# nathanaelbosch/ODEFilters.jl

Hardware: AMD Instinct MI355X
Metric: ensemble ODE-filter steps/sec (whole node) (higher is better)
Workload: dtype f64

## Files before the change

### odefilters.jl_amd/csrc/smooth_lane.h

```cpp
#pragma once
#include "ek_lane.h"

namespace odef {

struct LaneMem {
  double* base;
  int stride;
  __device__ inline double get(int k) const { return base[k * stride]; }
  __device__ inline void set(int k, double v) const { base[k * stride] = v; }
};

template <int D>
__device__ inline void two_sided_inverse(double (&S)[D * (D + 1) / 2], const double (&L)[D * (D + 1) / 2], const double (&dinv)[D]) {
  static_for<0, D>([&](auto kc) {
    constexpr int k = decltype(kc)::value;
    const double inv = dinv[k];
    const double tkk = S[tri(k, k)] * inv * inv;
    S[tri(k, k)] = tkk;
    const double htkk = -0.5 * tkk;
#pragma unroll
    for (int j = 0; j < k; ++j) S[tri(k, j)] *= inv;
    double b[D];
#pragma unroll
    for (int i = k + 1; i < D; ++i) {
      const double lik = L[tri(i, k)];
      b[i] = __builtin_fma(lik, htkk, S[tri(i, k)] * inv);
#pragma unroll
      for (int j = 0; j < k; ++j) S[tri(i, j)] = __builtin_fma(-lik, S[tri(k, j)], S[tri(i, j)]);
    }
#pragma unroll
    for (int i = k + 1; i < D; ++i) {
      const double lik = L[tri(i, k)];
#pragma unroll
      for (int j = k + 1; j <= i; ++j)
        S[tri(i, j)] = __builtin_fma(-L[tri(j, k)], b[i], __builtin_fma(-lik, b[j], S[tri(i, j)]));
      S[tri(i, k)] = __builtin_fma(lik, htkk, b[i]);
    }
    ODEF_SCHED_FENCE();
  });
  static_for<0, D>([&](auto kc) {
    constexpr int k = D - 1 - decltype(kc)::value;
    const double inv = dinv[k];
    double t[D];
#pragma unroll
    for (int j = 0; j < D; ++j) {
      double s = S[symidx(k, j)];
#pragma unroll
      for (int i = k + 1; i < D; ++i) s -= L[tri(i, k)] * S[symidx(i, j)];
      t[j] = s;
    }
    double tk = t[k];
#pragma unroll
    for (int i = k + 1; i < D; ++i) tk -= L[tri(i, k)] * t[i];
#pragma unroll
    for (int j = 0; j < D; ++j)
      if (j != k) S[symidx(k, j)] = t[j] * inv;
    S[tri(k, k)] = tk * inv * inv;
    ODEF_SCHED_FENCE();
  });
}

template <int d, int NB>
__device__ inline void congruence_At_inplace(const PriorConsts& pc, double (&X)[d * NB * (d * NB + 1) / 2]) {
  constexpr int D = d * NB;
#pragma unroll
  for (int J = NB - 1; J >= 1; --J) {
    double Wd[d][d];
#pragma unroll
    for (int a = 0; a < d; ++a)
#pragma unroll
      for (int b = 0; b < d; ++b) {
        double t = X[symidx(J * d + a, J * d + b)];
#pragma unroll
        for (int j = 0; j < J; ++j) t += pc.At[j][J] * X[symidx(j * d + a, J * d + b)];
        Wd[a][b] = t;
      }
#pragma unroll
    for (int a = 0; a < d; ++a)
#pragma unroll
      for (int c = 0; c < D; ++c) {
        if (c / d == J) continue;
        double t = X[symidx(J * d + a, c)];
#pragma unroll
        for (int j = 0; j < J; ++j) t += pc.At[j][J] * X[symidx(j * d + a, c)];
        X[symidx(J * d + a, c)] = t;
      }
#pragma unroll
    for (int a = 0; a < d; ++a)
#pragma unroll
      for (int b = 0; b <= a; ++b) {
        double t = Wd[a][b];
#pragma unroll
        for (int j = 0; j < J; ++j) t += pc.At[j][J] * X[symidx(J * d + a, j * d + b)];
        X[tri(J * d + a, J * d + b)] = t;
      }
  }
}

template <int d, int NB, class CovSink, class Sig = double>
__device__ inline void rts_step_core(const PriorConsts& pc, const double (&pij)[NB], const double (&mt)[d * NB],
                                     double (&B)[d * NB * (d * NB + 1) / 2], double (&Cs)[d * NB * (d * NB + 1) / 2],
                                     const double (&msn)[d * NB], Sig sigma2, const LaneMem& xl,
                                     double (&ms_out)[d * NB], CovSink& sink) {
  constexpr int D = d * NB, TRI = D * (D + 1) / 2;
  double dl[D];
#pragma unroll
  for (int J = 0; J < NB; ++J)
#pragma unroll
    for (int a = 0; a < d; ++a) {
      double t = mt[J * d + a];
#pragma unroll
      for (int j = J + 1; j < NB; ++j) t += pc.At[J][j] * mt[j * d + a];
      dl[J * d + a] = msn[J * d + a] - t;
    }
  ODEF_SCHED_FENCE();
  predict_cov_inplace<d, NB>(pc, B, sigma2);
  ODEF_SCHED_FENCE();
#pragma unroll
  for (int k = 0; k < TRI; ++k) Cs[k] -= B[k];
  int fixes = 0;
  double dinv[D];
  chol_packed<D>(B, fixes, dinv);
  ODEF_SCHED_FENCE();
#pragma unroll
  for (int k = 0; k < D; ++k) {
    double t = dl[k];
#pragma unroll
    for (int c = 0; c < k; ++c) t -= B[tri(k, c)] * dl[c];
    dl[k] = t * dinv[k];
  }
#pragma unroll
  for (int k = D - 1; k >= 0; --k) {
    double t = dl[k];
#pragma unroll
    for (int c = k + 1; c < D; ++c) t -= B[tri(c, k)] * dl[c];
    dl[k] = t * dinv[k];
  }
  double wv[D];
#pragma unroll
  for (int K = 0; K < NB; ++K)
#pragma unroll
    for (int b = 0; b < d; ++b) {
      double t = dl[K * d + b];
#pragma unroll
      for (int j = 0; j < K; ++j) t += pc.At[j][K] * dl[j * d + b];
      wv[K * d + b] = t;
    }
  ODEF_SCHED_FENCE();
  two_sided_inverse<D>(Cs, B, dinv);
  ODEF_SCHED_FENCE();
  congruence_At_inplace<d, NB>(pc, Cs);
  ODEF_SCHED_FENCE();
  static_for<0, D>([&](auto ac) {
    constexpr int a = decltype(ac)::value;
    double xa[D], u[D];
#pragma unroll
    for (int c = 0; c < D; ++c) xa[c] = xl.get(symidx(a, c));
    double mnew = mt[a];
#pragma unroll
    for (int c = 0; c < D; ++c) mnew += xa[c] * wv[c];
    ms_out[a] = mnew * pij[a / d];
#pragma unroll
    for (int c = 0; c < D; ++c) {
      double t = 0.0;
#pragma unroll
      for (int k = 0; k < D; ++k) t += xa[k] * Cs[symidx(k, c)];
      u[c] = t;
    }
#pragma unroll
    for (int b = 0; b <= a; ++b) {
      double t = xa[b];
#pragma unroll
      for (int k = 0; k < D; ++k) t += u[k] * xl.get(symidx(k, b));
      sink(tri(a, b), t * (pij[a / d] * pij[b / d]));
    }
    ODEF_SCHED_FENCE();
  });
}

__device__ inline long wave_uniform_max(long v, bool valid) {
#ifdef ODEF_HOST_EMUL
  (void)valid;
  return v;
#else
  int x = valid ? (int)v : 0;
  for (int m = 32; m >= 1; m >>= 1) {
    const int y = __shfl_xor(x, m, 64);
    x = x > y ? x : y;
  }
  return (long)__builtin_amdgcn_readfirstlane(x);
#endif
}

#ifdef ODEF_HOST_EMUL
inline double* agpr_file() {
  static thread_local double f[256];
  return f;
}
template <int R>
inline void aput(double v) { agpr_file()[R] = v; }
template <int R>
inline double aget() { return agpr_file()[R]; }
inline void agpr_file_claim() {}
#else
template <int R>
__device__ __attribute__((always_inline)) inline void aput(double v) {
  static_assert(R >= 0 && R < 128, "a lane has 256 AGPRs = 128 doubles");
  asm volatile("v_accvgpr_write_b32 a[%1], %0" ::"v"(__double2loint(v)), "n"(2 * R));
  asm volatile("v_accvgpr_write_b32 a[%1], %0" ::"v"(__double2hiint(v)), "n"(2 * R + 1));
}
template <int R>
__device__ __attribute__((always_inline)) inline double aget() {
  static_assert(R >= 0 && R < 128, "a lane has 256 AGPRs = 128 doubles");
  int lo, hi;
  asm volatile("v_accvgpr_read_b32 %0, a[%1]" : "=v"(lo) : "n"(2 * R));
  asm volatile("v_accvgpr_read_b32 %0, a[%1]" : "=v"(hi) : "n"(2 * R + 1));
  return __hiloint2double(hi, lo);
}
__device__ __attribute__((always_inline)) inline void agpr_file_claim() { asm volatile("" ::: "a255"); }
#endif

template <int n>
__device__ __attribute__((always_inline)) inline void pin(double (&a)[n]) {
#ifndef ODEF_HOST_EMUL
#pragma unroll
  for (int k = 0; k < n; ++k) asm volatile("" : "+v"(a[k]));
#else
  (void)a;
#endif
}

template <int D>
__device__ inline void ldl_packed_lane(double (&B)[D * (D + 1) / 2], double (&dinv)[D]) {
  static_for<0, D>([&](auto kc) {
    constexpr int k = decltype(kc)::value;
    const double piv = B[tri(k, k)];
    const bool ok = piv > 0.0;
    const double inv = ok ? rcp_pos(ok ? piv : 1.0) : 0.0;
    dinv[k] = inv;
    double v[D];
#pragma unroll
    for (int i = k + 1; i < D; ++i) {
      v[i] = B[tri(i, k)];
      B[tri(i, k)] = v[i] * inv;
    }
#pragma unroll
    for (int j = k + 1; j < D; ++j)
#pragma unroll
      for (int i = j; i < D; ++i) B[tri(i, j)] = __builtin_fma(-B[tri(i, k)], v[j], B[tri(i, j)]);
  });
}

template <int D, int LS>
__device__ inline void two_sided_inverse_parked(double (&S)[D * (D + 1) / 2]) {
  static_for<0, D>([&](auto kc) {
    constexpr int k = decltype(kc)::value;
    double lc[D];
    static_for<k + 1, D>([&](auto ic) { lc[decltype(ic)::value] = aget<LS + tri(decltype(ic)::value, k)>(); });
    const double htkk = -0.5 * S[tri(k, k)];
    double b[D];
#pragma unroll
    for (int i = k + 1; i < D; ++i) {
      b[i] = __builtin_fma(lc[i], htkk, S[tri(i, k)]);
#pragma unroll
      for (int j = 0; j < k; ++j) S[tri(i, j)] = __builtin_fma(-lc[i], S[tri(k, j)], S[tri(i, j)]);
    }
#pragma unroll
    for (int i = k + 1; i < D; ++i) {
#pragma unroll
      for (int j = k + 1; j <= i; ++j) S[tri(i, j)] = __builtin_fma(-lc[j], b[i], __builtin_fma(-lc[i], b[j], S[tri(i, j)]));
      S[tri(i, k)] = __builtin_fma(lc[i], htkk, b[i]);
    }
    pin(S);
    ODEF_SCHED_FENCE();
  });
  {
    double di[D];
    static_for<0, D>([&](auto kc) { di[decltype(kc)::value] = aget<LS + tri(decltype(kc)::value, decltype(kc)::value)>(); });
#pragma unroll
    for (int i = 0; i < D; ++i) {
#pragma unroll
      for (int j = 0; j < i; ++j) S[tri(i, j)] = (S[tri(i, j)] * di[i]) * di[j];
      S[tri(i, i)] = __builtin_fma(S[tri(i, i)] * di[i], di[i], -di[i]);
    }
    pin(S);
    ODEF_SCHED_FENCE();
  }
  static_for<0, D>([&](auto kc) {
    constexpr int k = D - 1 - decltype(kc)::value;
    double lc[D];
    static_for<k + 1, D>([&](auto ic) { lc[decltype(ic)::value] = aget<LS + tri(decltype(ic)::value, k)>(); });
    double t[D];
#pragma unroll
    for (int j = 0; j < D; ++j) {
      double s = S[symidx(k, j)];
#pragma unroll
      for (int i = k + 1; i < D; ++i) s -= lc[i] * S[symidx(i, j)];
      t[j] = s;
    }
    double tk = t[k];
#pragma unroll
    for (int i = k + 1; i < D; ++i) tk -= lc[i] * t[i];
#pragma unroll
    for (int j = 0; j < D; ++j)
      if (j != k) S[symidx(k, j)] = t[j];
    S[tri(k, k)] = tk;
    pin(S);
    ODEF_SCHED_FENCE();
  });
}

template <int d, int q, bool ADAPT>
__device__ inline void smooth_lane_v2(const SmoothParams& P, long i0, unsigned lane, const LaneMem& xl, long n_hi) {
  constexpr int NB = q + 1, D = d * NB, TRI = D * (D + 1) / 2;
  constexpr int MS = 128 - (TRI + D), VS = MS + TRI;
  static_assert(MS >= 0, "the AGPR file holds 128 doubles");
  agpr_file_claim();
  const long i = i0 + lane;
  const long n = ADAPT ? (long)P.nsaved[i] : P.n_save;
  const size_t N = (size_t)P.N;
  const PriorConsts& pc = P.pc;
  for (int w = 0; w < 2; ++w) {
    const long s = w == 0 ? 0 : n - 1;
    double c[TRI], m[D];
    const double* src = P.cov + ((size_t)s * TRI) * N + i;
#pragma unroll
    for (int k = 0; k < TRI; ++k) c[k] = src[(size_t)k * N];
#pragma unroll
    for (int k = 0; k < D; ++k) m[k] = P.mean[((size_t)s * D + k) * N + i];
    ODEF_SCHED_FENCE();
    double* dst = P.scov + ((size_t)s * TRI) * N + i;
#pragma unroll
    for (int k = 0; k < TRI; ++k) dst[(size_t)k * N] = c[k];
#pragma unroll
    for (int k = 0; k < D; ++k) P.smean[((size_t)s * D + k) * N + i] = m[k];
    static_for<0, TRI>([&](auto kc) { aput<MS + decltype(kc)::value>(c[decltype(kc)::value]); });
    static_for<0, D>([&](auto kc) { aput<VS + decltype(kc)::value>(m[decltype(kc)::value]); });
  }
  bool nan_seen = false;
  for (long s = n_hi - 2; s >= 1; --s) {
    if constexpr (ADAPT) {
      if (s > n - 2) continue;
    }
    double h, pj[NB], pij[NB];
    if constexpr (ADAPT) {
      h = P.tsave[(size_t)(s + 1) * N + i] - P.tsave[(size_t)s * N + i];
      double val = (h != 0.0) ? precond_val<q>(h) : 1.0;
#pragma unroll
      for (int J = 0; J < NB; ++J) {
        pj[J] = val;
        pij[J] = 1.0 / val;
        val *= h;
      }
    } else {
      h = uniform_load(P.hs + s);
      const GlobalTab tab{P.ptab + (size_t)uniform_load(P.tab_idx + s) * kTabStride};
#pragma unroll
      for (int J = 0; J < NB; ++J) {
        pj[J] = tab[kTabPJ + J];
        pij[J] = tab[kTabPIJ + J];
      }
    }
    RowStore sm(P.smean + ((size_t)s * D) * N + i0, N, D, lane), sc(P.scov + ((size_t)s * TRI) * N + i0, N, TRI, lane);
    if (h == 0.0) {
      static_for<0, D>([&](auto kc) { sm.put(aget<VS + decltype(kc)::value>()); });
      static_for<0, TRI>([&](auto kc) { sc.put(aget<MS + decltype(kc)::value>()); });
      continue;
    }
    const double sigma2 = P.diff[(size_t)(s + 1) * N + i];
    double mt[D], B[TRI];
    {
      RowLoad lc(P.cov + ((size_t)s * TRI) * N + i0, N, TRI, lane), lm(P.mean + ((size_t)s * D) * N + i0, N, D, lane);
#pragma unroll
      for (int k = 0; k < TRI; ++k) B[k] = lc.get();
#pragma unroll
      for (int k = 0; k < D; ++k) mt[k] = lm.get();
    }
    ODEF_SCHED_FENCE();
#pragma unroll
    for (int k = 0; k < D; ++k) mt[k] *= pj[k / d];
#pragma unroll
    for (int a = 0; a < D; ++a)
#pragma unroll
      for (int b = 0; b <= a; ++b) {
        const double x = B[tri(a, b)] * (pj[a / d] * pj[b / d]);
        xl.set(tri(a, b), x);
        B[tri(a, b)] = x;
      }
    pin(B);
    double dl[D];
    static_for<0, D>([&](auto kc) { dl[decltype(kc)::value] = aget<VS + decltype(kc)::value>(); });
#pragma unroll
    for (int J = 0; J < NB; ++J)
#pragma unroll
      for (int a = 0; a < d; ++a) {
        double t = mt[J * d + a];
#pragma unroll
        for (int j = J + 1; j < NB; ++j) t += pc.At[J][j] * mt[j * d + a];
        dl[J * d + a] = pj[J] * dl[J * d + a] - t;
      }
    pin(dl);
    ODEF_SCHED_FENCE();
    predict_cov_inplace<d, NB>(pc, B, sigma2);
    pin(B);
    ODEF_SCHED_FENCE();
    double dinv[D];
    ldl_packed_lane<D>(B, dinv);
    pin(B);
    pin(dinv);
    ODEF_SCHED_FENCE();
#pragma unroll
    for (int k = 0; k < D; ++k) {
      double t = dl[k];
#pragma unroll
      for (int c = 0; c < k; ++c) t -= B[tri(k, c)] * dl[c];
      dl[k] = t;
    }
#pragma unroll
    for (int k = 0; k < D; ++k) dl[k] *= dinv[k];
#pragma unroll
    for (int k = D - 1; k >= 0; --k) {
      double t = dl[k];
#pragma unroll
      for (int c = k + 1; c < D; ++c) t -= B[tri(c, k)] * dl[c];
      dl[k] = t;
    }
#pragma unroll
    for (int K = NB - 1; K >= 1; --K)
#pragma unroll
      for (int b = 0; b < d; ++b)
#pragma unroll
        for (int j = 0; j < K; ++j) dl[K * d + b] += pc.At[j][K] * dl[j * d + b];
#pragma unroll
    for (int a = 0; a < D; ++a)
#pragma unroll
      for (int c = 0; c <= a; ++c) {
        const double x = xl.get(tri(a, c));
        mt[a] += x * dl[c];
        if (c != a) mt[c] += x * dl[a];
      }
    static_for<0, D>([&](auto kc) {
      constexpr int k = decltype(kc)::value;
      const double v = mt[k] * pij[k / d];
      nan_seen = nan_seen || !(v == v);
      sm.put(v);
      aput<VS + k>(v);
    });
    ODEF_SCHED_FENCE();
    double S[TRI];
    static_for<0, TRI>([&](auto kc) {
      constexpr int k = decltype(kc)::value;
      constexpr int a = [] { int r = 0; while ((r + 1) * (r + 2) / 2 <= k) ++r; return r; }();
      constexpr int b = k - a * (a + 1) / 2;
      S[k] = aget<MS + k>();
      aput<MS + k>(a == b ? dinv[a] : B[k]);
      S[k] *= pj[a / d] * pj[b / d];
    });
    pin(S);
    ODEF_SCHED_FENCE();
    two_sided_inverse_parked<D, MS>(S);
    pin(S);
    ODEF_SCHED_FENCE();
    congruence_At_inplace<d, NB>(pc, S);
    pin(S);
    ODEF_SCHED_FENCE();
    auto rows = [&](auto a0c, auto nrc) {
      constexpr int a0 = decltype(a0c)::value, nr = decltype(nrc)::value;
      double u[nr][D];
#pragma unroll
      for (int r = 0; r < nr; ++r) {
        double xa[D];
#pragma unroll
        for (int c = 0; c < D; ++c) xa[c] = xl.get(symidx(a0 + r, c));
#pragma unroll
        for (int c = 0; c < D; ++c) {
          double t = 0.0;
#pragma unroll
          for (int k = 0; k < D; ++k) t += xa[k] * S[symidx(k, c)];
          u[r][c] = t;
        }
      }
      RowStore st[2] = {sc.at_row(tri(a0, 0)), sc.at_row(tri(a0 + nr - 1, 0))};
      static_for<0, a0 + nr>([&](auto bc) {
        constexpr int b = decltype(bc)::value;
        double col[D];
#pragma unroll
        for (int k = 0; k < D; ++k) col[k] = xl.get(symidx(k, b));
        static_for<0, nr>([&](auto rc) {
          constexpr int a = a0 + decltype(rc)::value;
          if constexpr (b <= a) {
            double t = col[a];
#pragma unroll
            for (int k = 0; k < D; ++k) t += u[a - a0][k] * col[k];
            const double v = t * (pij[a / d] * pij[b / d]);
            st[a - a0].put(v);
            aput<MS + tri(a, b)>(v);
          }
        });
      });
      ODEF_SCHED_FENCE();
    };
    static_for<0, D / 2>([&](auto pc_) { rows(std::integral_constant<int, 2 * decltype(pc_)::value>{}, std::integral_constant<int, 2>{}); });
    if constexpr (D % 2 == 1) rows(std::integral_constant<int, D - 1>{}, std::integral_constant<int, 1>{});
  }
  if (nan_seen) P.retcode[i] = 3;
}

}
```

Before: 7.445 billion.

## Reformulate RTS smoother step using inverse transition to drop forward prediction

The smoother step now forms the prediction in the reversed time direction. It adds a sign-flipped process noise Q instead of running the full A·P·Aᵀ prediction congruence, and it applies the transition inverse (reversed A) to the smoothed covariance before the two-sided inverse rather than applying Aᵀ afterwards. The mean update is rewritten to use the inverse transition on the residual and to accumulate a correction that is fused into the final scaling with an FMA. This removes one dense congruence and a back-propagation loop per step. It relies on the algebraic identity of the reversed transition, which could change rounding behaviour and numerical stability in f64.

```diff
diff --git a/odefilters.jl_amd/csrc/smooth_lane.h b/odefilters.jl_amd/csrc/smooth_lane.h
--- a/odefilters.jl_amd/csrc/smooth_lane.h
+++ b/odefilters.jl_amd/csrc/smooth_lane.h
@@ -95,6 +95,56 @@
         X[tri(J * d + a, J * d + b)] = t;
       }
   }
+}
+
+__device__ inline double reversed_At(const PriorConsts& pc, int J, int j) { return ((j - J) & 1) ? -pc.At[J][j] : pc.At[J][j]; }
+
+template <int d, int NB>
+__device__ inline void congruence_Ainv_inplace(const PriorConsts& pc, double (&X)[d * NB * (d * NB + 1) / 2]) {
+  constexpr int D = d * NB;
+#pragma unroll
+  for (int J = 0; J + 1 < NB; ++J) {
+    double Wd[d][d];
+#pragma unroll
+    for (int a = 0; a < d; ++a)
+#pragma unroll
+      for (int b = 0; b < d; ++b) {
+        double t = X[symidx(J * d + a, J * d + b)];
+#pragma unroll
+        for (int j = J + 1; j < NB; ++j) t += reversed_At(pc, J, j) * X[symidx(j * d + a, J * d + b)];
+        Wd[a][b] = t;
+      }
+#pragma unroll
+    for (int a = 0; a < d; ++a)
+#pragma unroll
+      for (int c = 0; c < D; ++c) {
+        if (c / d == J) continue;
+        double t = X[symidx(J * d + a, c)];
+#pragma unroll
+        for (int j = J + 1; j < NB; ++j) t += reversed_At(pc, J, j) * X[symidx(j * d + a, c)];
+        X[symidx(J * d + a, c)] = t;
+      }
+#pragma unroll
+    for (int a = 0; a < d; ++a)
+#pragma unroll
+      for (int b = 0; b <= a; ++b) {
+        double t = Wd[a][b];
+#pragma unroll
+        for (int j = J + 1; j < NB; ++j) t += reversed_At(pc, J, j) * X[symidx(J * d + a, j * d + b)];
+        X[tri(J * d + a, J * d + b)] = t;
+      }
+  }
+}
+
+template <int d, int NB, class Sig>
+__device__ inline void add_reversed_Q(const PriorConsts& pc, double (&B)[d * NB * (d * NB + 1) / 2], Sig sigma2) {
+#pragma unroll
+  for (int J = 0; J < NB; ++J)
+#pragma unroll
+    for (int K = 0; K <= J; ++K)
+#pragma unroll
+      for (int a = 0; a < d; ++a)
+        B[tri(J * d + a, K * d + a)] += sig_comp(sigma2, a) * (((J + K) & 1) ? -pc.Qt[J][K] : pc.Qt[J][K]);
 }
 
 template <int d, int NB, class CovSink, class Sig = double>
@@ -378,8 +428,6 @@
     }
     ODEF_SCHED_FENCE();
 #pragma unroll
-    for (int k = 0; k < D; ++k) mt[k] *= pj[k / d];
-#pragma unroll
     for (int a = 0; a < D; ++a)
 #pragma unroll
       for (int b = 0; b <= a; ++b) {
@@ -391,17 +439,19 @@
     double dl[D];
     static_for<0, D>([&](auto kc) { dl[decltype(kc)::value] = aget<VS + decltype(kc)::value>(); });
 #pragma unroll
+    for (int k = 0; k < D; ++k) dl[k] *= pj[k / d];
+#pragma unroll
     for (int J = 0; J < NB; ++J)
 #pragma unroll
       for (int a = 0; a < d; ++a) {
-        double t = mt[J * d + a];
-#pragma unroll
-        for (int j = J + 1; j < NB; ++j) t += pc.At[J][j] * mt[j * d + a];
-        dl[J * d + a] = pj[J] * dl[J * d + a] - t;
+        double t = dl[J * d + a];
+#pragma unroll
+        for (int j = J + 1; j < NB; ++j) t += reversed_At(pc, J, j) * dl[j * d + a];
+        dl[J * d + a] = __builtin_fma(-pj[J], mt[J * d + a], t);
       }
     pin(dl);
     ODEF_SCHED_FENCE();
-    predict_cov_inplace<d, NB>(pc, B, sigma2);
+    add_reversed_Q<d, NB>(pc, B, sigma2);
     pin(B);
     ODEF_SCHED_FENCE();
     double dinv[D];
@@ -425,23 +475,20 @@
       for (int c = k + 1; c < D; ++c) t -= B[tri(c, k)] * dl[c];
       dl[k] = t;
     }
-#pragma unroll
-    for (int K = NB - 1; K >= 1; --K)
-#pragma unroll
-      for (int b = 0; b < d; ++b)
-#pragma unroll
-        for (int j = 0; j < K; ++j) dl[K * d + b] += pc.At[j][K] * dl[j * d + b];
+    double xw[D];
+#pragma unroll
+    for (int a = 0; a < D; ++a) xw[a] = 0.0;
 #pragma unroll
     for (int a = 0; a < D; ++a)
 #pragma unroll
       for (int c = 0; c <= a; ++c) {
         const double x = xl.get(tri(a, c));
-        mt[a] += x * dl[c];
-        if (c != a) mt[c] += x * dl[a];
+        xw[a] += x * dl[c];
+        if (c != a) xw[c] += x * dl[a];
       }
     static_for<0, D>([&](auto kc) {
       constexpr int k = decltype(kc)::value;
-      const double v = mt[k] * pij[k / d];
+      const double v = __builtin_fma(xw[k], pij[k / d], mt[k]);
       nan_seen = nan_seen || !(v == v);
       sm.put(v);
       aput<VS + k>(v);
@@ -458,10 +505,10 @@
     });
     pin(S);
     ODEF_SCHED_FENCE();
+    congruence_Ainv_inplace<d, NB>(pc, S);
+    pin(S);
+    ODEF_SCHED_FENCE();
     two_sided_inverse_parked<D, MS>(S);
-    pin(S);
-    ODEF_SCHED_FENCE();
-    congruence_At_inplace<d, NB>(pc, S);
     pin(S);
     ODEF_SCHED_FENCE();
     auto rows = [&](auto a0c, auto nrc) {
```

Result: no change. 7.484 billion, median of 2 (+0.5%).
